# 4m4n5/CLIP-Lite

Hardware: AMD Instinct MI355X
Metric: image-caption pairs/sec (global batch) — ResNet-50+BERT bs1024, 1/2/4/8 MI355X (higher is better)
Workload: dtype bf16; 1 GPU; resnet50 + BERT-base(12L) + JSD-MI heads/priors, per-GPU batch 128, 224x224 images, 30-token captions, dropout 0.1 + prior noise on, clip 10 + SGD(0.9, wd 1e-4) + Lookahead(5, 0.5); global_batch=128, parallelism=dp1

## Files before the change

### clip-lite_amd/bert.py

```python
import torch
import torch.nn as nn

from . import hip


class LinearParams(nn.Module):
    def __init__(self, cin, cout, bias=True, std=None):
        super().__init__()
        self.in_features, self.out_features = cin, cout
        self.weight = nn.Parameter(torch.empty(cout, cin))
        self.bias = nn.Parameter(torch.zeros(cout)) if bias else None
        if std is None:
            nn.init.kaiming_uniform_(self.weight, a=5 ** 0.5)
            if bias:
                bound = 1 / cin ** 0.5
                nn.init.uniform_(self.bias, -bound, bound)
        else:
            self.weight.data.normal_(0.0, std)


class LayerNormParams(nn.Module):
    def __init__(self, c, eps):
        super().__init__()
        self.normalized_shape, self.eps = (c,), eps
# ... 274 lines not shown
        ds2 = _alloc(rt, M, Hd)
        ds2m = _alloc(rt, M, Hd) if d2[0] > 0 else None
        hip.layernorm_bwd(dt, dh, s2, st2, out.LayerNorm.weight, ds2, ds2m, A.g(out.LayerNorm.weight), A.g(out.LayerNorm.bias), M, Hd, drop_out=d2,
                          dcolsum=A.g(out.dense.bias))
        dz2 = ds2m if ds2m is not None else ds2
        _linear_grads(rt, out.dense, dz2, g, M, bias_done=True, defer=defer)
        df = _alloc(rt, M, inner)
        ib = layer.intermediate.dense.bias
        fold = ib is not None and ib.requires_grad
        _dgrad(rt, dz2, M, inner, Hd, hip.epilogue(df, inner, dact_aux=f, dact=hip.DACT_GELU, colsum=A.g(ib) if fold else None, colsum_rows=1),
               out.dense.weight)
        _linear_grads(rt, layer.intermediate.dense, df, h1, M, bias_done=fold, defer=defer)
        dh1 = _alloc(rt, M, Hd)
        _dgrad(rt, df, M, Hd, inner, hip.epilogue(dh1, Hd, residual=ds2), layer.intermediate.dense.weight)
        ds1 = _alloc(rt, M, Hd)
        ds1m = _alloc(rt, M, Hd) if d1[0] > 0 else None
        hip.layernorm_bwd(dt, dh1, s1, st1, ln1.weight, ds1, ds1m, A.g(ln1.weight), A.g(ln1.bias), M, Hd, drop_out=d1,
                          dcolsum=A.g(wo.bias))
        dz1 = ds1m if ds1m is not None else ds1
        _linear_grads(rt, wo, dz1, ctxt, M, bias_done=True, defer=defer)
        dctx = _alloc(rt, M, Hd)
        _dgrad(rt, dz1, M, Hd, Hd, hip.epilogue(dctx, Hd), wo.weight)
        dqkv = _alloc(rt, M, 3 * Hd)
        if mp:
            n_part = B * heads * 32
            hip.attention_bias_bwd(dt, qkv, ctx["mask"], ctx["bias"], net.bucket_table, dctx, dqkv, ctx["dbias_partials"][li * n_part:(li + 1) * n_part],
                                   B, L, heads, da)
        else:
            hip.attention_bwd(dt, qkv, ctx["mask"], dctx, dqkv, B, L, heads, da)
        _linear_grads(rt, None, dqkv, h, M, dw=A.span([wq.weight, wk.weight, wv.weight], grad=True).view(3 * Hd, Hd),
                      db=A.span([wq.bias, wk.bias, wv.bias], grad=True), defer=defer)
        dhp = _alloc(rt, M, Hd)
        _dgrad(rt, dqkv, M, Hd, 3 * Hd, hip.epilogue(dhp, Hd, residual=ds1), wq.weight, wk.weight, wv.weight)
        dh = dhp
        if own_group is None:
            rt.grads_ready(layer)
        elif staged:
            own_group.launch()
            if not pooler_done:
                rt.grads_ready(net.pooler)
                pooler_done = True
            rt.grads_ready(layer)
            defer = own_group = hip.WgradGroup(rt.dt)
    if not last:
        ctx["bwd_dh"] = dh
        return
    emb = net.embeddings
    ds0 = _alloc(rt, M, Hd)
    if mp:
        rel = net.encoder.relative_attention_bias.weight
        if nl and rel.requires_grad:
            hip.attention_bias_grad_reduce(ctx["dbias_partials"], A.g(rel), nl * B, heads)
        if own_group is None or staged:
            rt.grads_ready(net.encoder.relative_attention_bias)
# ... 18 lines not shown
```

### clip-lite_amd/csrc/bert_ops.hip

```cpp
#include "vec.h"
#include "rng.h"
#include "det.h"
#include "clite.h"

using namespace clite;

namespace {

constexpr int LN_MAXCH = 4;

struct Drop { float p; uint64_t seed; uint32_t site; };

DEV void apply_dropout8(const Drop& d, size_t idx, float (&v)[8]) {
  float u[8];
  dropout_uniform8(d.seed, d.site, idx, u);
  float ks = 1.0f / (1.0f - d.p);
#pragma unroll
  for (int e = 0; e < 8; ++e) v[e] = u[e] >= d.p ? v[e] * ks : 0.f;
}

struct LnQ8 { uint8_t* out; const float* scale; float* amax; };
template <typename T, int NCH, bool Q = false>
__global__ __launch_bounds__(256) void layernorm_fwd_kernel(const T* x, const float* gamma, const float* beta, float eps, T* out,
                                                            float* stats, int M, int C, Drop drop, LnQ8 q8) {
// ... 474 lines not shown
      dk += sm.dS[t * AT_PP + r] * sm.f.q[t * AT_PQ + lane];
      dv += sm.f.p[t * AT_PP + r] * sm.f.m[t * AT_PP + r] * sm.dO[t * AT_PQ + lane];
    }
    dq *= 0.125f; dk *= 0.125f;
    T* o = obase + (size_t)r * ld + lane;
    if constexpr (sizeof(T) == 2) { o[0] = f2bf(dq); o[H * AT_D] = f2bf(dk); o[2 * H * AT_D] = f2bf(dv); }
    else { o[0] = dq; o[H * AT_D] = dk; o[2 * H * AT_D] = dv; }
  }
}
constexpr int AM_PI = 192;
constexpr int AM_PT = 80;

struct AmFwdSmem { char v[32 * AM_PI]; float madd[32]; };
struct AmBwdSmem { char q[32 * AM_PI], k[32 * AM_PI], d[32 * AM_PI], t[32 * AM_PT]; float m[32 * 33]; float madd[32]; };

DEV void am_load_image(const bf16* base, size_t ld, int L, char* img, int lane) {
  for (int c = lane; c < 256; c += 64) {
    int r = c >> 3, ch = c & 7;
    u32x4 v = {0u, 0u, 0u, 0u};
    if (r < L) v = *(const u32x4*)(base + (size_t)r * ld + ch * 8);
    *(u32x4*)(img + r * AM_PI + ch * 16) = v;
  }
}
DEV bf16x8 am_frag_rows(const bf16* base, size_t ld, int L, int ks, int lane) {
  Chunk16 c;
  c.u = u32x4{0u, 0u, 0u, 0u};
  int r = lane & 31;
  if (r < L) c.u = *(const u32x4*)(base + (size_t)r * ld + ks * 16 + 8 * (lane >> 5));
  return c.h;
}
template <int PITCH> DEV bf16x8 am_frag_tr(const char* img, int x0, int s, int lane) {
  int x = x0 + 16 * ((lane >> 4) & 1) + 4 * (lane & 3);
  int k = 16 * s + 8 * (lane >> 5) + ((lane >> 2) & 3);
  const char* p = img + k * PITCH + x * 2;
  union { s16x4 v[2]; bf16x8 h; } u;
  u.v[0] = lds_read_tr16(p);
  u.v[1] = lds_read_tr16(p + 4 * PITCH);
  return u.h;
}
template <int PITCH> DEV bf16x8 am_frag_tr_acc(const char* img, int x0, int s, int lane) {
  int x = x0 + 16 * ((lane >> 4) & 1) + 4 * (lane & 3);
  int k = 16 * s + 4 * (lane >> 5) + ((lane >> 2) & 3);
  const char* p = img + k * PITCH + x * 2;
  union { s16x4 v[2]; bf16x8 h; } u;
  u.v[0] = lds_read_tr16(p);
  u.v[1] = lds_read_tr16(p + 8 * PITCH);
  return u.h;
}
DEV bf16x8 am_acc_frag(const f32x16& a, int s) {
  bf16x8 f;
#pragma unroll
  for (int e = 0; e < 8; ++e) f[e] = f2bf(a[8 * s + e]);
  return f;
}
DEV int am_row(int r, int lane) { return (r & 3) + 8 * (r >> 2) + 4 * (lane >> 5); }
DEV void am_store_T(bf16* base, size_t ld, int L, int d0, const f32x16& a, float scale, int lane) {
  int tok = lane & 31;
  if (tok >= L) return;
#pragma unroll
  for (int g = 0; g < 4; ++g) {
    union { bf16 e[4]; u32x2 u; } pk;
#pragma unroll
    for (int e = 0; e < 4; ++e) pk.e[e] = f2bf(a[4 * g + e] * scale);
    *(u32x2*)(base + (size_t)tok * ld + d0 + 8 * g + 4 * (lane >> 5)) = pk.u;
  }
}

template <bool BIAS = false>
__global__ __launch_bounds__(256) void attention_mfma_fwd_kernel(const bf16* qkv, const int64_t* mask, bf16* ctx, int B, int L, int H, Drop drop, AttnBias<BIAS> ab) {
  seed_resolve(drop.seed, drop.site);
  __shared__ __attribute__((aligned(16))) AmFwdSmem sm[4];
  const int lane = threadIdx.x & 63, wave = threadIdx.x >> 6;
  int bh = blockIdx.x * 4 + wave;
  const bool live = bh < B * H;
  if (!live) bh = B * H - 1;
  const int b = bh / H, h = bh % H;
  const size_t ld = (size_t)3 * H * 64;
  const bf16* qb = qkv + (size_t)b * L * ld + h * 64;
  AmFwdSmem& S = sm[wave];
  am_load_image(qb + 2 * H * 64, ld, L, S.v, lane);
  if (lane < 32) S.madd[lane] = (lane < L) ? ((mask && mask[(size_t)b * L + lane] == 0) ? AT_NEG : 0.f) : -INFINITY;
  f32x16 acc;
#pragma unroll
  for (int r = 0; r < 16; ++r) acc[r] = 0.f;
#pragma unroll
  for (int ks = 0; ks < 4; ++ks)
    acc = mfma32_bf16(am_frag_rows(qb + H * 64, ld, L, ks, lane), am_frag_rows(qb, ld, L, ks, lane), acc);
// ... 11 lines not shown
  for (int r = 0; r < 16; ++r) { acc[r] = __expf(acc[r] - mx); den += acc[r]; }
  den += wave_shfl_xor(den, 32);
  const float inv = 1.0f / den;
  const int i = lane & 31;
#pragma unroll
  for (int g = 0; g < 4; ++g) {
    float u[4] = {1.f, 1.f, 1.f, 1.f};
    if (drop.p > 0.f) rng_uniform4(drop.seed, drop.site, ((size_t)bh * AT_L + i) * AT_L + 8 * g + 4 * (lane >> 5), u);
    const float ks = drop.p > 0.f ? 1.0f / (1.0f - drop.p) : 1.f;
#pragma unroll
    for (int e = 0; e < 4; ++e) acc[4 * g + e] *= inv * (u[e] >= drop.p ? ks : 0.f);
  }
#pragma unroll
  for (int db = 0; db < 2; ++db) {
    f32x16 o;
#pragma unroll
    for (int r = 0; r < 16; ++r) o[r] = 0.f;
#pragma unroll
    for (int s = 0; s < 2; ++s) o = mfma32_bf16(am_frag_tr_acc<AM_PI>(S.v, db * 32, s, lane), am_acc_frag(acc, s), o);
    if (live) am_store_T(ctx + (size_t)b * L * ((size_t)H * 64) + h * 64, (size_t)H * 64, L, db * 32, o, 1.f, lane);
  }
}
template <bool BIAS = false>
__global__ __launch_bounds__(128) void attention_mfma_bwd_kernel(const bf16* qkv, const int64_t* mask, const bf16* dctx, bf16* dqkv, int B, int L, int H, Drop drop,
                                                                 AttnBias<BIAS> ab) {
  seed_resolve(drop.seed, drop.site);
  __shared__ __attribute__((aligned(16))) AmBwdSmem sm[2];
  const int lane = threadIdx.x & 63, wave = threadIdx.x >> 6;
  int bh = blockIdx.x * 2 + wave;
  const bool live = bh < B * H;
  if (!live) bh = B * H - 1;
  const int b = bh / H, h = bh % H;
  const size_t ld = (size_t)3 * H * 64, ldc = (size_t)H * 64;
  const bf16* qb = qkv + (size_t)b * L * ld + h * 64;
  const bf16* dob = dctx + (size_t)b * L * ldc + h * 64;
  AmBwdSmem& S = sm[wave];
  am_load_image(qb, ld, L, S.q, lane);
  am_load_image(qb + H * 64, ld, L, S.k, lane);
  am_load_image(dob, ldc, L, S.d, lane);
  if (lane < 32) S.madd[lane] = (lane < L) ? ((mask && mask[(size_t)b * L + lane] == 0) ? AT_NEG : 0.f) : -INFINITY;
  {
    const float ks = drop.p > 0.f ? 1.0f / (1.0f - drop.p) : 1.f;
    for (int q4 = lane; q4 < 256; q4 += 64) {
      int i = q4 >> 3, j0 = (q4 & 7) * 4;
      float u[4] = {1.f, 1.f, 1.f, 1.f};
      if (drop.p > 0.f) rng_uniform4(drop.seed, drop.site, ((size_t)bh * AT_L + i) * AT_L + j0, u);
#pragma unroll
      for (int e = 0; e < 4; ++e) S.m[i * 33 + j0 + e] = u[e] >= drop.p ? ks : 0.f;
    }
  }
  f32x16 p, dp;
#pragma unroll
  for (int r = 0; r < 16; ++r) { p[r] = 0.f; dp[r] = 0.f; }
#pragma unroll
  for (int ks = 0; ks < 4; ++ks) {
    p = mfma32_bf16(am_frag_rows(qb, ld, L, ks, lane), am_frag_rows(qb + H * 64, ld, L, ks, lane), p);
    dp = mfma32_bf16(am_frag_rows(dob, ldc, L, ks, lane), am_frag_rows(qb + 2 * H * 64, ld, L, ks, lane), dp);
  }
  __syncthreads();
  const int j = lane & 31;
  const float madd = S.madd[j];
  f32x16 pd, ds;
#pragma unroll
  for (int r = 0; r < 16; ++r) {
    float s;
    if constexpr (BIAS) s = (p[r] * 0.125f + ab.bias[((size_t)h * AT_L + am_row(r, lane)) * AT_L + j]) + madd;
    else s = p[r] * 0.125f + madd;
    float mx = s;
#pragma unroll
    for (int m = 16; m >= 1; m >>= 1) mx = fmaxf(mx, wave_shfl_xor(mx, m));
    float e = __expf(s - mx);
    float den = e;
#pragma unroll
    for (int m = 16; m >= 1; m >>= 1) den += wave_shfl_xor(den, m);
    int i = am_row(r, lane);
    float pr = (i < L) ? e / den : 0.f;
    float mul = S.m[i * 33 + j];
    float dpd = dp[r] * mul;
    float t = dpd * pr;
#pragma unroll
    for (int m = 16; m >= 1; m >>= 1) t += wave_shfl_xor(t, m);
    p[r] = pr;
    pd[r] = pr * mul;
    ds[r] = pr * (dpd - t);
  }
  if constexpr (BIAS) {
#pragma unroll
    for (int r = 0; r < 16; ++r) S.m[am_row(r, lane) * 33 + j] = ds[r];
  }
#pragma unroll
  for (int g = 0; g < 4; ++g) {
    union { bf16 e[4]; u32x2 u; } pk;
#pragma unroll
    for (int e = 0; e < 4; ++e) pk.e[e] = f2bf(ds[4 * g + e]);
    *(u32x2*)(S.t + j * AM_PT + (8 * g + 4 * (lane >> 5)) * 2) = pk.u;
  }
  __syncthreads();
  if constexpr (BIAS) attn_bucket_sums(S.m, 33, L, ab.btab, live ? ab.partials + (size_t)bh * AT_L : nullptr, lane);
  bf16* ob = dqkv + (size_t)b * L * ld + h * 64;
#pragma unroll
  for (int db = 0; db < 2; ++db) {
    f32x16 dv, dk, dq;
#pragma unroll
    for (int r = 0; r < 16; ++r) { dv[r] = 0.f; dk[r] = 0.f; dq[r] = 0.f; }
#pragma unroll
    for (int s = 0; s < 2; ++s) {
      dv = mfma32_bf16(am_frag_tr_acc<AM_PI>(S.d, db * 32, s, lane), am_acc_frag(pd, s), dv);
      dk = mfma32_bf16(am_frag_tr_acc<AM_PI>(S.q, db * 32, s, lane), am_acc_frag(ds, s), dk);
      dq = mfma32_bf16(am_frag_tr<AM_PI>(S.k, db * 32, s, lane), am_frag_tr<AM_PT>(S.t, 0, s, lane), dq);
    }
    if (live) {
      am_store_T(ob + 2 * H * 64, ld, L, db * 32, dv, 1.f, lane);
      am_store_T(ob + H * 64, ld, L, db * 32, dk, 0.125f, lane);
      am_store_T(ob, ld, L, db * 32, dq, 0.125f, lane);
    }
  }
}
__global__ __launch_bounds__(256) void attention_bias_build_kernel(const float* rel, const int32_t* btab, float* bias, int H, int L) {
  const int idx = blockIdx.x * 256 + threadIdx.x;
  if (idx >= H * AT_L * AT_L) return;
  const int h = idx / (AT_L * AT_L), i = (idx / AT_L) % AT_L, j = idx % AT_L;
  float v = 0.f;
  if (i < L && j < L) {
    int k = btab[j - i + AT_L - 1];
    k = k < 0 ? 0 : (k > AT_L - 1 ? AT_L - 1 : k);
    v = rel[k * H + h];
  }
  bias[idx] = v;
}
__global__ __launch_bounds__(1024) void attention_bias_grad_reduce_kernel(const float* partials, float* drel, int R, int H) {
  __shared__ float red[32][33];
  const int h = blockIdx.x, k = threadIdx.x & 31, part = threadIdx.x >> 5;
  float acc = 0.f;
  for (int r = part; r < R; r += 32) acc += partials[((size_t)r * H + h) * AT_L + k];
  red[part][k] = acc;
  __syncthreads();
  if (threadIdx.x < 32) {
    float t = 0.f;
// ... 447 lines not shown
           hipLaunchKernelGGL(embed_bwd_kernel<float>, dim3(egrid), dim3(128), 0, st, ids, (const float*)d, dword, dpos, M / L, L, C, vocab, padding_idx, EmbMp<false>{}));
  return (int)hipGetLastError();
}

extern "C" int clite_attention_fwd(int dtype, const void* qkv, const int64_t* mask, void* ctx, int B, int L, int H,
                                   float drop_p, uint64_t drop_seed, uint32_t drop_site, void* stream) {
  if (B <= 0 || L <= 0 || L > AL_L || H <= 0 || !qkv || !ctx) return -1;
  Drop d{drop_p, drop_seed, drop_site};
  hipStream_t st = (hipStream_t)stream;
  if (L > AT_L) {
#define AL_FWD(NT) hipLaunchKernelGGL(attention_long_mfma_fwd_kernel<NT>, dim3(B * H), dim3(64 * NT), 0, st, (const bf16*)qkv, mask, (bf16*)ctx, B, L, H, d)
    DISPATCH(dtype,
             if (L <= 64) AL_FWD(2); else if (L <= 96) AL_FWD(3); else AL_FWD(4),
             hipLaunchKernelGGL(attention_long_fwd_kernel<float>, dim3(B * H), dim3(256), 0, st, (const float*)qkv, mask, (float*)ctx, B, L, H, d));
#undef AL_FWD
    return (int)hipGetLastError();
  }
  DISPATCH(dtype,
           hipLaunchKernelGGL(attention_mfma_fwd_kernel<false>, dim3((B * H + 3) / 4), dim3(256), 0, st, (const bf16*)qkv, mask, (bf16*)ctx, B, L, H, d, AttnBias<false>{}),
           hipLaunchKernelGGL(attention_fwd_kernel<float>, dim3(B * H), dim3(64), 0, st, (const float*)qkv, mask, (float*)ctx, B, L, H, d, AttnBias<false>{}));
  return (int)hipGetLastError();
}

extern "C" int clite_attention_bwd(int dtype, const void* qkv, const int64_t* mask, const void* dctx, void* dqkv, int B, int L, int H,
                                   float drop_p, uint64_t drop_seed, uint32_t drop_site, void* stream) {
  if (B <= 0 || L <= 0 || L > AL_L || H <= 0 || !qkv || !dctx || !dqkv) return -1;
  Drop d{drop_p, drop_seed, drop_site};
  hipStream_t st = (hipStream_t)stream;
  if (L > AT_L) {
#define AL_BWD(NT) hipLaunchKernelGGL(attention_long_mfma_bwd_kernel<NT>, dim3(B * H), dim3(64 * NT), 0, st, (const bf16*)qkv, mask, (const bf16*)dctx, (bf16*)dqkv, B, L, H, d)
    DISPATCH(dtype,
             if (L <= 64) AL_BWD(2); else if (L <= 96) AL_BWD(3); else AL_BWD(4),
             hipLaunchKernelGGL(attention_long_bwd_kernel<float>, dim3(B * H), dim3(256), 0, st, (const float*)qkv, mask, (const float*)dctx, (float*)dqkv, B, L, H, d));
#undef AL_BWD
    return (int)hipGetLastError();
  }
  DISPATCH(dtype,
           hipLaunchKernelGGL(attention_mfma_bwd_kernel<false>, dim3((B * H + 1) / 2), dim3(128), 0, st, (const bf16*)qkv, mask, (const bf16*)dctx, (bf16*)dqkv, B, L, H, d, AttnBias<false>{}),
           hipLaunchKernelGGL(attention_bwd_kernel<float>, dim3(B * H), dim3(64), 0, st, (const float*)qkv, mask, (const float*)dctx, (float*)dqkv, B, L, H, d, AttnBias<false>{}));
  return (int)hipGetLastError();
}

extern "C" int clite_attention_bias_fwd(int dtype, const void* qkv, const int64_t* mask, const float* bias, void* ctx, int B, int L, int H,
                                        float drop_p, uint64_t drop_seed, uint32_t drop_site, void* stream) {
  if (B <= 0 || L <= 0 || L > AT_L || H <= 0 || !qkv || !ctx || !bias) return -1;
  Drop d{drop_p, drop_seed, drop_site};
  AttnBias<true> ab{bias, nullptr, nullptr};
  hipStream_t st = (hipStream_t)stream;
  DISPATCH(dtype,
           hipLaunchKernelGGL(attention_mfma_fwd_kernel<true>, dim3((B * H + 3) / 4), dim3(256), 0, st, (const bf16*)qkv, mask, (bf16*)ctx, B, L, H, d, ab),
           hipLaunchKernelGGL((attention_fwd_kernel<float, true>), dim3(B * H), dim3(64), 0, st, (const float*)qkv, mask, (float*)ctx, B, L, H, d, ab));
  return (int)hipGetLastError();
}

extern "C" int clite_attention_bias_bwd(int dtype, const void* qkv, const int64_t* mask, const float* bias, const int32_t* bucket_table, const void* dctx,
                                        void* dqkv, float* dbias_partials, int B, int L, int H, float drop_p, uint64_t drop_seed, uint32_t drop_site,
                                        void* stream) {
  if (B <= 0 || L <= 0 || L > AT_L || H <= 0 || !qkv || !dctx || !dqkv || !bias || !bucket_table || !dbias_partials) return -1;
  Drop d{drop_p, drop_seed, drop_site};
  AttnBias<true> ab{bias, bucket_table, dbias_partials};
  hipStream_t st = (hipStream_t)stream;
  DISPATCH(dtype,
           hipLaunchKernelGGL(attention_mfma_bwd_kernel<true>, dim3((B * H + 1) / 2), dim3(128), 0, st, (const bf16*)qkv, mask, (const bf16*)dctx, (bf16*)dqkv, B, L, H, d, ab),
           hipLaunchKernelGGL((attention_bwd_kernel<float, true>), dim3(B * H), dim3(64), 0, st, (const float*)qkv, mask, (const float*)dctx, (float*)dqkv, B, L, H, d, ab));
  return (int)hipGetLastError();
}

extern "C" int clite_attention_bias_build(const float* rel_weight, const int32_t* bucket_table, float* bias, int H, int L, void* stream) {
  if (H <= 0 || L <= 0 || L > AT_L || !rel_weight || !bucket_table || !bias) return -1;
  hipLaunchKernelGGL(attention_bias_build_kernel, dim3((H * AT_L * AT_L + 255) / 256), dim3(256), 0, (hipStream_t)stream, rel_weight, bucket_table, bias, H, L);
  return (int)hipGetLastError();
}

extern "C" int clite_attention_bias_grad_reduce(const float* partials, float* drel, int rows, int H, void* stream) {
  if (rows <= 0 || H <= 0 || !partials || !drel) return -1;
  hipLaunchKernelGGL(attention_bias_grad_reduce_kernel, dim3(H), dim3(1024), 0, (hipStream_t)stream, partials, drel, rows, H);
  return (int)hipGetLastError();
}

extern "C" int clite_embed_mpnet_fwd(int dtype, const int64_t* ids, const void* word, const void* pos, void* out, int32_t* pids, int M, int L, int C,
                                     int vocab, int max_pos, int padding_idx, void* stream) {
  if (M <= 0 || L <= 0 || L > 32 || M % L || C % 8 || vocab <= 0 || max_pos <= 0 || !ids || !word || !pos || !out) return -1;
  int grid = (M + 3) / 4;
  if (grid > 4096) grid = 4096;
  hipStream_t st = (hipStream_t)stream;
  DISPATCH(dtype,
           hipLaunchKernelGGL(embed_mpnet_fwd_kernel<bf16>, dim3(grid), dim3(256), 0, st, ids, (const bf16*)word, (const bf16*)pos, (bf16*)out, pids, M, L, C, vocab, max_pos, padding_idx),
           hipLaunchKernelGGL(embed_mpnet_fwd_kernel<float>, dim3(grid), dim3(256), 0, st, ids, (const float*)word, (const float*)pos, (float*)out, pids, M, L, C, vocab, max_pos, padding_idx));
// ... 46 lines not shown
```

### clip-lite_amd/hip.py

```python
import ctypes as C
import os

import torch

_HERE = os.path.dirname(os.path.abspath(__file__))
LIB_PATH = os.environ.get("CLITE_HIP_LIB") or os.path.join(_HERE, "lib", "libclite_hip.so")
ABI_VERSION = 12

BF16, F32 = 0, 1
ACT_NONE, ACT_RELU, ACT_GELU, ACT_TANH = 0, 1, 2, 3
DACT_RELU, DACT_GELU, DACT_TANH = 1, 2, 3
SEED_INDIRECT = 0x80000000

TORCH_DTYPE = {BF16: torch.bfloat16, F32: torch.float32}


class Epilogue(C.Structure):
    _fields_ = [
        ("out", C.c_void_p), ("ldc", C.c_int32), ("out_f32", C.c_int32), ("atomic", C.c_int32),
        ("alpha", C.c_float), ("bias", C.c_void_p), ("act", C.c_int32), ("preact", C.c_void_p),
        ("dact_aux", C.c_void_p), ("dact", C.c_int32), ("drop_p", C.c_float), ("drop_seed", C.c_uint64),
        ("drop_site", C.c_uint32), ("residual", C.c_void_p), ("colsum", C.c_void_p),
        ("colsum_replicas", C.c_int32), ("colsum_stride", C.c_int32), ("colsum_rows", C.c_int32),
        ("bn_y", C.c_void_p), ("bn_stats", C.c_void_p), ("bn_replicas", C.c_int32), ("bn_rstride", C.c_int32),
# ... 85 lines not shown
    "clite_stem_pack": [_V, _V, _I, _V],
    "clite_stem_unpack_grad": [_V, _V, _V],
    "clite_bn_apply": [_V, _I, _V, _V, _V, _V],
    "clite_bn_centered_var": [_I, _V, _V, _I, _I, _I, _I, _V],
    "clite_bn_bwd_reduce": [_I, _V, _V, _V, _V, _V, _V, _I, _I, _I, _I, _V],
    "clite_bn_bwd_apply": [_V, _I, _V, _V, _V, _V, _V, _V, _V, _V, _V, _V],
    "clite_maxpool3x3s2_fwd": [_I, _V, _V, _V, _I, _I, _I, _I, _V],
    "clite_maxpool3x3s2_bwd": [_I, _V, _V, _V, _I, _I, _I, _I, _V],
    "clite_stem_bn_pool_fwd": [_V, _I, _V, _V, _V, _I, _I, _I, _V],
    "clite_stem_bn_pool_bwd": [_V, _I, _V, _V, _V, _V, _V, _V, _V, _I, _I, _I, _V],
    "clite_stem_bn_pool_fwd_ex": [_V, _I, _V, _V, _V, _V, _I, _I, _I, _V],
    "clite_stem_bn_pool_bwd_apply": [_V, _I, _V, _V, _V, _V, _V, _V, _V, _I, _I, _I, _V],
    "clite_avgpool_fwd": [_I, _V, _V, _I, _I, _I, _V],
    "clite_avgpool_bwd": [_I, _V, _V, _I, _I, _I, _V],
    "clite_image_to_nhwc4": [_I, _V, _V, _I, _I, _I, _I, _I, _I, _V],
    "clite_colsum": [_I, _V, _V, _I, _I, _V],
    "clite_layernorm_fwd": [_I, _V, _V, _V, _F, _V, _V, _I, _I, _F, _U64, _U32, _V],
    "clite_layernorm_fwd_q8": [_I, _V, _V, _V, _F, _V, _V, _I, _I, _F, _U64, _U32, _V, _V, _V, _V],
    "clite_layernorm_bwd": [_I, _V, _V, _V, _V, _V, _V, _V, _V, _V, _I, _I, _F, _U64, _U32, _F, _U64, _U32, _V],
    "clite_embed_fwd": [_I, _V, _V, _V, _V, _V, _I, _I, _I, _I, _V],
    "clite_embed_bwd": [_I, _V, _V, _V, _V, _I, _I, _I, _I, _I, _V],
    "clite_attention_fwd": [_I, _V, _V, _V, _I, _I, _I, _F, _U64, _U32, _V],
    "clite_attention_bwd": [_I, _V, _V, _V, _V, _I, _I, _I, _F, _U64, _U32, _V],
    "clite_attention_bias_fwd": [_I, _V, _V, _V, _V, _I, _I, _I, _F, _U64, _U32, _V],
    "clite_attention_bias_bwd": [_I, _V, _V, _V, _V, _V, _V, _V, _I, _I, _I, _F, _U64, _U32, _V],
    "clite_attention_bias_build": [_V, _V, _V, _I, _I, _V],
    "clite_attention_bias_grad_reduce": [_V, _V, _I, _I, _V],
    "clite_embed_mpnet_fwd": [_I, _V, _V, _V, _V, _V, _I, _I, _I, _I, _I, _I, _V],
    "clite_embed_mpnet_bwd": [_I, _V, _V, _V, _V, _V, _I, _I, _I, _I, _I, _I, _V],
    "clite_mean_pool_fwd": [_I, _V, _V, _V, _V, _I, _I, _I, _V],
    "clite_mean_pool_bwd": [_I, _V, _V, _V, _V, _I, _I, _I, _V],
    "clite_tanh_bwd": [_I, _V, _V, _V, _U64, _V],
    "clite_critic_jsd_fwd": [_I, _V, _V, _V, _I, _I, _V, _V, _V, _V],
    "clite_l2_normalize": [_I, _V, _V, _I, _I, _V],
    "clite_l2_normalize_bwd": [_I, _V, _V, _V, _V, _I, _I, _V],
    "clite_infonce_fwd": [_V, _I, _I, _V, _V, _V, _V, _V],
    "clite_infonce_bwd": [_I, _V, _I, _I, _V, _V, _V, _V, _F, _V, _I, _V, _V],
    "clite_xent_fwd": [_V, _I, _I, _I, _V, _I, _V, _V, _V],
    "clite_xent_bwd": [_I, _V, _I, _I, _I, _I, _V, _V, _V, _V, _V, _I, _V],
    "clite_svm_margin": [_V, _V, _V, _I, _I, _I, _V, _V, _V, _V, _V],
    "clite_svm_hess_scale": [_V, _V, _U64, _V],
    "clite_svm_newton_begin": [_V, _I, _I, _I, _V, _V, _V, _V, _F, _I, _F, _V],
    "clite_svm_cg_update": [_V, _I, _I, _I, _V, _V, _V, _V, _V],
    "clite_svm_line_search": [_V, _V, _V, _V, _I, _I, _I, _V, _V, _I, _I, _V, _V],
    "clite_average_precision": [_V, _I, _V, _I, _I, _I, _V, _V],
    "clite_retrieval_rank_i2t": [_V, _I, _I, _I, _V, _V, _V, _V],
    "clite_retrieval_rank_t2i": [_V, _I, _I, _I, _V, _V, _V, _V],
    "clite_kmeans_row_norms": [_V, _I, _I, _I, _F, _V, _V],
# ... 570 lines not shown
                                           p(fp8[0]), p(fp8[1]), p(fp8[2]), stream_ptr(x)), "layernorm_fwd_q8")
        return
    check(lib().clite_layernorm_fwd(dt, p(x), p(gamma), p(beta), eps, p(out), p(stats), M, Cc, drop[0], drop[1], drop[2], stream_ptr(x)),
          "layernorm_fwd")


def layernorm_bwd(dt, dy, x, stats, gamma, dx, dx_masked, dgamma, dbeta, M, Cc, drop_in=NO_DROP, drop_out=NO_DROP, dcolsum=None):
    check(lib().clite_layernorm_bwd(dt, p(dy), p(x), p(stats), p(gamma), p(dx), p(dx_masked), p(dgamma), p(dbeta), p(dcolsum), M, Cc,
                                    drop_in[0], drop_in[1], drop_in[2], drop_out[0], drop_out[1], drop_out[2], stream_ptr(x)), "layernorm_bwd")


def embed_fwd(dt, ids, word, pos, typ, out, M, L, Cc, vocab):
    check(lib().clite_embed_fwd(dt, p(ids), p(word), p(pos), p(typ), p(out), M, L, Cc, vocab, stream_ptr(out)), "embed_fwd")


def embed_bwd(dt, ids, d, dword, dpos, M, L, Cc, vocab, padding_idx=-1):
    check(lib().clite_embed_bwd(dt, p(ids), p(d), p(dword), p(dpos), M, L, Cc, vocab, padding_idx, stream_ptr(d)), "embed_bwd")


def attention_fwd(dt, qkv, mask, ctx, B, L, H, drop=NO_DROP):
    check(lib().clite_attention_fwd(dt, p(qkv), p(mask), p(ctx), B, L, H, drop[0], drop[1], drop[2], stream_ptr(qkv)), "attention_fwd")


def attention_bwd(dt, qkv, mask, dctx, dqkv, B, L, H, drop=NO_DROP):
    check(lib().clite_attention_bwd(dt, p(qkv), p(mask), p(dctx), p(dqkv), B, L, H, drop[0], drop[1], drop[2], stream_ptr(qkv)), "attention_bwd")


def relative_position_buckets(num_buckets=32, max_distance=128, span=31):
    half = num_buckets // 2
    exact = half // 2
    assert (num_buckets, max_distance) == (32, 128), "the closed form below is for MPNetConfig's defaults"
    out = []
    for rel in range(-span, span + 1):
        n = -rel
        ret = half if n < 0 else 0
        n = abs(n)
        if n < exact:
            ret += n
        else:
            t = 0
            while 2 ** (t + 1) * exact * exact <= n * n:
                t += 1
            ret += min(exact + t, half - 1)
        out.append(ret)
    return out


def attention_bias_fwd(dt, qkv, mask, bias, ctx, B, L, H, drop=NO_DROP):
    check(lib().clite_attention_bias_fwd(dt, p(qkv), p(mask), p(bias), p(ctx), B, L, H, drop[0], drop[1], drop[2], stream_ptr(qkv)), "attention_bias_fwd")


def attention_bias_bwd(dt, qkv, mask, bias, table, dctx, dqkv, partials, B, L, H, drop=NO_DROP):
    assert partials.dtype == torch.float32 and partials.numel() >= B * H * 32 and table.dtype == torch.int32 and table.numel() == 63
    check(lib().clite_attention_bias_bwd(dt, p(qkv), p(mask), p(bias), p(table), p(dctx), p(dqkv), p(partials), B, L, H, drop[0], drop[1], drop[2],
                                         stream_ptr(qkv)), "attention_bias_bwd")


def attention_bias_build(rel_weight, table, bias, H, L):
    assert rel_weight.dtype == torch.float32 and tuple(rel_weight.shape) == (32, H) and bias.dtype == torch.float32 and bias.numel() == H * 1024
    assert table.dtype == torch.int32 and table.numel() == 63
    check(lib().clite_attention_bias_build(p(rel_weight), p(table), p(bias), H, L, stream_ptr(bias)), "attention_bias_build")


def attention_bias_grad_reduce(partials, drel, rows, H):
    assert partials.numel() >= rows * H * 32 and drel.dtype == torch.float32 and drel.numel() == 32 * H
    check(lib().clite_attention_bias_grad_reduce(p(partials), p(drel), rows, H, stream_ptr(partials)), "attention_bias_grad_reduce")


def embed_mpnet_fwd(dt, ids, word, pos, out, pids, M, L, Cc, vocab, max_pos, padding_idx):
    check(lib().clite_embed_mpnet_fwd(dt, p(ids), p(word), p(pos), p(out), p(pids), M, L, Cc, vocab, max_pos, padding_idx, stream_ptr(out)), "embed_mpnet_fwd")


def embed_mpnet_bwd(dt, ids, pids, d, dword, dpos, M, L, Cc, vocab, max_pos, padding_idx):
    check(lib().clite_embed_mpnet_bwd(dt, p(ids), p(pids), p(d), p(dword), p(dpos), M, L, Cc, vocab, max_pos, padding_idx, stream_ptr(d)), "embed_mpnet_bwd")


def mean_pool_fwd(dt, h, mask, out, inv, B, L, Cc):
    check(lib().clite_mean_pool_fwd(dt, p(h), p(mask), p(out), p(inv), B, L, Cc, stream_ptr(out)), "mean_pool_fwd")
# ... 271 lines not shown
```

### include/clite.h

```cpp
#ifndef CLITE_H
#define CLITE_H
#include <stdint.h>

#ifdef __cplusplus
extern "C" {
#endif

#define CLITE_ABI_VERSION 12
int clite_abi_version(void);

int clite_set_deterministic(int on);
int clite_get_deterministic(void);

int clite_set_f32_split(int on);
int clite_get_f32_split(void);

int clite_set_tile_policy(int policy);

enum { CLITE_BF16 = 0, CLITE_F32 = 1 };

#define CLITE_SEED_INDIRECT 0x80000000u

enum { CLITE_ACT_NONE = 0, CLITE_ACT_RELU = 1, CLITE_ACT_GELU = 2, CLITE_ACT_TANH = 3 };

// ... 182 lines not shown
int clite_stem_bn_pool_bwd_apply(const clite_bn* p, int dtype, const void* dpool, const uint8_t* idx, const void* y, const float* dstats, void* dy,
                                 float* dgamma, float* dbeta, int N, int H, int W, void* stream);
int clite_avgpool_fwd(int dtype, const void* x, void* out, int N, int HW, int C, void* stream);
int clite_avgpool_bwd(int dtype, const void* dout, void* dx, int N, int HW, int C, void* stream);
int clite_image_to_nhwc4(int dtype, const float* img, void* out, int N, int H, int W, int pad, int Hp, int Wp, void* stream);
int clite_colsum(int dtype, const void* x, float* out, int M, int N, void* stream);

int clite_layernorm_fwd(int dtype, const void* x, const float* gamma, const float* beta, float eps, void* out, float* stats,
                        int M, int C, float drop_p, uint64_t drop_seed, uint32_t drop_site, void* stream);
int clite_layernorm_fwd_q8(int dtype, const void* x, const float* gamma, const float* beta, float eps, void* out, float* stats,
                           int M, int C, float drop_p, uint64_t drop_seed, uint32_t drop_site, uint8_t* fp8_out, const float* fp8_scale, float* fp8_amax,
                           void* stream);
int clite_layernorm_bwd(int dtype, const void* dy, const void* x, const float* stats, const float* gamma, void* dx, void* dx_masked,
                        float* dgamma, float* dbeta, float* dcolsum, int M, int C, float in_p, uint64_t in_seed, uint32_t in_site,
                        float out_p, uint64_t out_seed, uint32_t out_site, void* stream);
int clite_embed_fwd(int dtype, const int64_t* ids, const void* word, const void* pos, const void* type, void* out,
                    int M, int L, int C, int vocab, void* stream);
int clite_embed_bwd(int dtype, const int64_t* ids, const void* d, float* dword, float* dpos, int M, int L, int C, int vocab, int padding_idx,
                    void* stream);
int clite_attention_fwd(int dtype, const void* qkv, const int64_t* mask, void* ctx, int B, int L, int H,
                        float drop_p, uint64_t drop_seed, uint32_t drop_site, void* stream);
int clite_attention_bwd(int dtype, const void* qkv, const int64_t* mask, const void* dctx, void* dqkv, int B, int L, int H,
                        float drop_p, uint64_t drop_seed, uint32_t drop_site, void* stream);

int clite_attention_bias_fwd(int dtype, const void* qkv, const int64_t* mask, const float* bias, void* ctx, int B, int L, int H,
                             float drop_p, uint64_t drop_seed, uint32_t drop_site, void* stream);
int clite_attention_bias_bwd(int dtype, const void* qkv, const int64_t* mask, const float* bias, const int32_t* bucket_table, const void* dctx,
                             void* dqkv, float* dbias_partials, int B, int L, int H, float drop_p, uint64_t drop_seed, uint32_t drop_site,
                             void* stream);
int clite_attention_bias_build(const float* rel_weight, const int32_t* bucket_table, float* bias, int H, int L, void* stream);
int clite_attention_bias_grad_reduce(const float* partials, float* drel, int rows, int H, void* stream);
int clite_embed_mpnet_fwd(int dtype, const int64_t* ids, const void* word, const void* pos, void* out, int32_t* pids, int M, int L, int C,
                          int vocab, int max_pos, int padding_idx, void* stream);
int clite_embed_mpnet_bwd(int dtype, const int64_t* ids, const int32_t* pids, const void* d, float* dword, float* dpos, int M, int L, int C,
                          int vocab, int max_pos, int padding_idx, void* stream);
int clite_mean_pool_fwd(int dtype, const void* h, const int64_t* mask, void* out, float* inv, int B, int L, int C, void* stream);
int clite_mean_pool_bwd(int dtype, const void* dy, const int64_t* mask, const float* inv, void* dh, int B, int L, int C, void* stream);

int clite_tanh_bwd(int dtype, const void* dy, const void* y, void* out, uint64_t n, void* stream);

int clite_critic_jsd_fwd(int dtype, const void* f1, const void* f2, const float* temperature, int B, int D, const int32_t* neg, float* work,
                         float* acc, void* stream);
int clite_l2_normalize(int dtype, const void* x, void* out, int B, int D, void* stream);
int clite_l2_normalize_bwd(int dtype, const void* x, const void* y, const void* dy, void* dx, int B, int D, void* stream);
int clite_infonce_fwd(const float* C, int ld, int B, const float* temperature, float* lse_r, float* lse_c, float* acc, void* stream);
int clite_infonce_bwd(int dtype, const float* C, int ld, int B, const float* temperature, const float* lse_r, const float* lse_c,
                      const float* gout, float scale, void* dC, int ldd, float* dtemp, void* stream);
int clite_critic_jsd_bwd(int dtype, const void* f1, const void* f2, const float* temperature, const float* work, const float* gout, float scale,
                         int B, int D, const int32_t* neg, const int32_t* neg_inv, void* df1, void* df2, float* dtemp, void* stream);
int clite_prior_tail_fwd(int dtype, const void* h1, const float* w2, const float* b2, int B, int K, int softplus, float* logit, float* acc,
                         void* stream);
int clite_prior_tail_bwd(int dtype, const void* h1, const float* w2, const float* logit, const float* gout, float scale, int B, int K,
// ... 98 lines not shown
```

Measured before the change: 8782 pairs/s.

## Fuse QKV bias-gradient reduction into attention backward kernel and prefetch operands

The attention backward kernel now stages the finished dQ/dK/dV tiles in LDS, sums them over tokens, and atomically adds the result into the fused QKV bias gradient. This lets the separate bias reduction in the linear-grad path be skipped. The kernel also prefetches Q, K, dO, V fragments, the mask and the bias values into registers before the dropout mask generation, then feeds the MFMAs from LDS images instead of re-reading global memory. This adds float atomics, which are non-deterministic, so the fused path is disabled in deterministic mode. It also raises register pressure.

Result: no change. 8841 pairs/s (median of 6 runs) (+0.7%).

```diff
diff --git a/clip-lite_amd/bert.py b/clip-lite_amd/bert.py
--- a/clip-lite_amd/bert.py
+++ b/clip-lite_amd/bert.py
@@ -320,14 +320,16 @@
         dctx = _alloc(rt, M, Hd)
         _dgrad(rt, dz1, M, Hd, Hd, hip.epilogue(dctx, Hd), wo.weight)
         dqkv = _alloc(rt, M, 3 * Hd)
+        qkv_db = A.span([wq.bias, wk.bias, wv.bias], grad=True)
+        fused_db = qkv_db is not None and hip.attention_dbias_applies(dt, L)
         if mp:
             n_part = B * heads * 32
             hip.attention_bias_bwd(dt, qkv, ctx["mask"], ctx["bias"], net.bucket_table, dctx, dqkv, ctx["dbias_partials"][li * n_part:(li + 1) * n_part],
-                                   B, L, heads, da)
-        else:
-            hip.attention_bwd(dt, qkv, ctx["mask"], dctx, dqkv, B, L, heads, da)
+                                   B, L, heads, da, dqkv_bias=qkv_db if fused_db else None)
+        else:
+            hip.attention_bwd(dt, qkv, ctx["mask"], dctx, dqkv, B, L, heads, da, dqkv_bias=qkv_db if fused_db else None)
         _linear_grads(rt, None, dqkv, h, M, dw=A.span([wq.weight, wk.weight, wv.weight], grad=True).view(3 * Hd, Hd),
-                      db=A.span([wq.bias, wk.bias, wv.bias], grad=True), defer=defer)
+                      db=None if fused_db else qkv_db, defer=defer)
         dhp = _alloc(rt, M, Hd)
         _dgrad(rt, dqkv, M, Hd, 3 * Hd, hip.epilogue(dhp, Hd, residual=ds1), wq.weight, wk.weight, wv.weight)
         dh = dhp
diff --git a/clip-lite_amd/csrc/bert_ops.hip b/clip-lite_amd/csrc/bert_ops.hip
--- a/clip-lite_amd/csrc/bert_ops.hip
+++ b/clip-lite_amd/csrc/bert_ops.hip
@@ -520,6 +520,34 @@
     *(u32x4*)(img + r * AM_PI + ch * 16) = v;
   }
 }
+DEV void am_fetch_image(const bf16* base, size_t ld, int L, u32x4 (&g)[4], int lane) {
+#pragma unroll
+  for (int n = 0; n < 4; ++n) {
+    int c = lane + 64 * n, r = c >> 3, ch = c & 7;
+    g[n] = *(const u32x4*)(base + (size_t)(r < L ? r : 0) * ld + ch * 8);
+  }
+}
+DEV void am_store_image(const u32x4 (&g)[4], int L, char* img, int lane) {
+#pragma unroll
+  for (int n = 0; n < 4; ++n) {
+    int c = lane + 64 * n, r = c >> 3;
+    *(u32x4*)(img + r * AM_PI + (c & 7) * 16) = r < L ? g[n] : u32x4{0u, 0u, 0u, 0u};
+  }
+}
+DEV u32x4 am_fetch_frag_rows(const bf16* base, size_t ld, int L, int ks, int lane) {
+  int r = lane & 31;
+  return *(const u32x4*)(base + (size_t)(r < L ? r : 0) * ld + ks * 16 + 8 * (lane >> 5));
+}
+DEV bf16x8 am_frag_fetched(u32x4 g, int L, int lane) {
+  Chunk16 c;
+  c.u = (lane & 31) < L ? g : u32x4{0u, 0u, 0u, 0u};
+  return c.h;
+}
+DEV bf16x8 am_frag_img(const char* img, int ks, int lane) {
+  Chunk16 c;
+  c.u = *(const u32x4*)(img + (lane & 31) * AM_PI + ks * 32 + 16 * (lane >> 5));
+  return c.h;
+}
 DEV bf16x8 am_frag_rows(const bf16* base, size_t ld, int L, int ks, int lane) {
   Chunk16 c;
   c.u = u32x4{0u, 0u, 0u, 0u};
@@ -561,6 +589,17 @@
 #pragma unroll
     for (int e = 0; e < 4; ++e) pk.e[e] = f2bf(a[4 * g + e] * scale);
     *(u32x2*)(base + (size_t)tok * ld + d0 + 8 * g + 4 * (lane >> 5)) = pk.u;
+  }
+}
+DEV void am_stash_T(char* img, int L, int d0, const f32x16& a, float scale, int lane) {
+  int tok = lane & 31;
+  if (tok >= L) return;
+#pragma unroll
+  for (int g = 0; g < 4; ++g) {
+    union { bf16 e[4]; u32x2 u; } pk;
+#pragma unroll
+    for (int e = 0; e < 4; ++e) pk.e[e] = f2bf(a[4 * g + e] * scale);
+    *(u32x2*)(img + tok * AM_PI + (d0 + 8 * g + 4 * (lane >> 5)) * 2) = pk.u;
   }
 }
 
@@ -618,8 +657,8 @@
   }
 }
 template <bool BIAS = false>
-__global__ __launch_bounds__(128) void attention_mfma_bwd_kernel(const bf16* qkv, const int64_t* mask, const bf16* dctx, bf16* dqkv, int B, int L, int H, Drop drop,
-                                                                 AttnBias<BIAS> ab) {
+__global__ __launch_bounds__(128) void attention_mfma_bwd_kernel(const bf16* qkv, const int64_t* mask, const bf16* dctx, bf16* dqkv, float* dqkv_bias, int B, int L,
+                                                                 int H, Drop drop, AttnBias<BIAS> ab) {
   seed_resolve(drop.seed, drop.site);
   __shared__ __attribute__((aligned(16))) AmBwdSmem sm[2];
   const int lane = threadIdx.x & 63, wave = threadIdx.x >> 6;
@@ -631,36 +670,59 @@
   const bf16* qb = qkv + (size_t)b * L * ld + h * 64;
   const bf16* dob = dctx + (size_t)b * L * ldc + h * 64;
   AmBwdSmem& S = sm[wave];
-  am_load_image(qb, ld, L, S.q, lane);
-  am_load_image(qb + H * 64, ld, L, S.k, lane);
-  am_load_image(dob, ldc, L, S.d, lane);
-  if (lane < 32) S.madd[lane] = (lane < L) ? ((mask && mask[(size_t)b * L + lane] == 0) ? AT_NEG : 0.f) : -INFINITY;
+  u32x4 gq[4], gk[4], gd[4];
+  am_fetch_image(qb, ld, L, gq, lane);
+  am_fetch_image(qb + H * 64, ld, L, gk, lane);
+  am_fetch_image(dob, ldc, L, gd, lane);
+  u32x4 gv[4];
+#pragma unroll
+  for (int ks = 0; ks < 4; ++ks) gv[ks] = am_fetch_frag_rows(qb + 2 * H * 64, ld, L, ks, lane);
+  u32x2 gm = {1u, 0u};
+  if (mask) gm = *(const u32x2*)(mask + (size_t)b * L + (lane < L ? lane : 0));
+  float bs[BIAS ? 16 : 1];
+  if constexpr (BIAS) {
+#pragma unroll
+    for (int r = 0; r < 16; ++r) bs[r] = ab.bias[((size_t)h * AT_L + am_row(r, lane)) * AT_L + (lane & 31)];
+  }
   {
     const float ks = drop.p > 0.f ? 1.0f / (1.0f - drop.p) : 1.f;
-    for (int q4 = lane; q4 < 256; q4 += 64) {
-      int i = q4 >> 3, j0 = (q4 & 7) * 4;
-      float u[4] = {1.f, 1.f, 1.f, 1.f};
-      if (drop.p > 0.f) rng_uniform4(drop.seed, drop.site, ((size_t)bh * AT_L + i) * AT_L + j0, u);
-#pragma unroll
-      for (int e = 0; e < 4; ++e) S.m[i * 33 + j0 + e] = u[e] >= drop.p ? ks : 0.f;
-    }
-  }
+    float u[4][4];
+#pragma unroll
+    for (int n = 0; n < 4; ++n) {
+      int q4 = lane + 64 * n, i = q4 >> 3, j0 = (q4 & 7) * 4;
+#pragma unroll
+      for (int e = 0; e < 4; ++e) u[n][e] = 1.f;
+      if (drop.p > 0.f) rng_uniform4(drop.seed, drop.site, ((size_t)bh * AT_L + i) * AT_L + j0, u[n]);
+    }
+#pragma unroll
+    for (int n = 0; n < 4; ++n) {
+      int q4 = lane + 64 * n, i = q4 >> 3, j0 = (q4 & 7) * 4;
+#pragma unroll
+      for (int e = 0; e < 4; ++e) S.m[i * 33 + j0 + e] = u[n][e] >= drop.p ? ks : 0.f;
+    }
+  }
+  am_store_image(gq, L, S.q, lane);
+  am_store_image(gk, L, S.k, lane);
+  am_store_image(gd, L, S.d, lane);
+  int m0 = (int)gm[0], m1 = (int)gm[1];
+  opaque_i(m0); opaque_i(m1);
+  if (lane < 32) S.madd[lane] = (lane < L) ? ((m0 | m1) == 0 ? AT_NEG : 0.f) : -INFINITY;
+  __syncthreads();
   f32x16 p, dp;
 #pragma unroll
   for (int r = 0; r < 16; ++r) { p[r] = 0.f; dp[r] = 0.f; }
 #pragma unroll
   for (int ks = 0; ks < 4; ++ks) {
-    p = mfma32_bf16(am_frag_rows(qb, ld, L, ks, lane), am_frag_rows(qb + H * 64, ld, L, ks, lane), p);
-    dp = mfma32_bf16(am_frag_rows(dob, ldc, L, ks, lane), am_frag_rows(qb + 2 * H * 64, ld, L, ks, lane), dp);
-  }
-  __syncthreads();
+    p = mfma32_bf16(am_frag_img(S.q, ks, lane), am_frag_img(S.k, ks, lane), p);
+    dp = mfma32_bf16(am_frag_img(S.d, ks, lane), am_frag_fetched(gv[ks], L, lane), dp);
+  }
   const int j = lane & 31;
   const float madd = S.madd[j];
   f32x16 pd, ds;
 #pragma unroll
   for (int r = 0; r < 16; ++r) {
     float s;
-    if constexpr (BIAS) s = (p[r] * 0.125f + ab.bias[((size_t)h * AT_L + am_row(r, lane)) * AT_L + j]) + madd;
+    if constexpr (BIAS) s = (p[r] * 0.125f + bs[r]) + madd;
     else s = p[r] * 0.125f + madd;
     float mx = s;
 #pragma unroll
@@ -694,22 +756,52 @@
   __syncthreads();
   if constexpr (BIAS) attn_bucket_sums(S.m, 33, L, ab.btab, live ? ab.partials + (size_t)bh * AT_L : nullptr, lane);
   bf16* ob = dqkv + (size_t)b * L * ld + h * 64;
+  f32x16 dv[2], dk[2], dq[2];
 #pragma unroll
   for (int db = 0; db < 2; ++db) {
-    f32x16 dv, dk, dq;
-#pragma unroll
-    for (int r = 0; r < 16; ++r) { dv[r] = 0.f; dk[r] = 0.f; dq[r] = 0.f; }
+#pragma unroll
+    for (int r = 0; r < 16; ++r) { dv[db][r] = 0.f; dk[db][r] = 0.f; dq[db][r] = 0.f; }
 #pragma unroll
     for (int s = 0; s < 2; ++s) {
-      dv = mfma32_bf16(am_frag_tr_acc<AM_PI>(S.d, db * 32, s, lane), am_acc_frag(pd, s), dv);
-      dk = mfma32_bf16(am_frag_tr_acc<AM_PI>(S.q, db * 32, s, lane), am_acc_frag(ds, s), dk);
-      dq = mfma32_bf16(am_frag_tr<AM_PI>(S.k, db * 32, s, lane), am_frag_tr<AM_PT>(S.t, 0, s, lane), dq);
+      dv[db] = mfma32_bf16(am_frag_tr_acc<AM_PI>(S.d, db * 32, s, lane), am_acc_frag(pd, s), dv[db]);
+      dk[db] = mfma32_bf16(am_frag_tr_acc<AM_PI>(S.q, db * 32, s, lane), am_acc_frag(ds, s), dk[db]);
+      dq[db] = mfma32_bf16(am_frag_tr<AM_PI>(S.k, db * 32, s, lane), am_frag_tr<AM_PT>(S.t, 0, s, lane), dq[db]);
     }
     if (live) {
-      am_store_T(ob + 2 * H * 64, ld, L, db * 32, dv, 1.f, lane);
-      am_store_T(ob + H * 64, ld, L, db * 32, dk, 0.125f, lane);
-      am_store_T(ob, ld, L, db * 32, dq, 0.125f, lane);
-    }
+      am_store_T(ob + 2 * H * 64, ld, L, db * 32, dv[db], 1.f, lane);
+      am_store_T(ob + H * 64, ld, L, db * 32, dk[db], 0.125f, lane);
+      am_store_T(ob, ld, L, db * 32, dq[db], 0.125f, lane);
+    }
+  }
+  if (!dqkv_bias) return;
+  lds_barrier();
+#pragma unroll
+  for (int db = 0; db < 2; ++db) {
+    am_stash_T(S.d, L, db * 32, dv[db], 1.f, lane);
+    am_stash_T(S.k, L, db * 32, dk[db], 0.125f, lane);
+    am_stash_T(S.q, L, db * 32, dq[db], 0.125f, lane);
+  }
+  lds_barrier();
+  float cs[3] = {0.f, 0.f, 0.f};
+  for (int t = 0; t < L; ++t) {
+    cs[0] += bf2f(*(const bf16*)(S.q + t * AM_PI + lane * 2));
+    cs[1] += bf2f(*(const bf16*)(S.k + t * AM_PI + lane * 2));
+    cs[2] += bf2f(*(const bf16*)(S.d + t * AM_PI + lane * 2));
+  }
+  if (H == 1) {
+    float* fold = sm[1].m;
+    if (wave == 1) {
+#pragma unroll
+      for (int w = 0; w < 3; ++w) fold[w * 64 + lane] = live ? cs[w] : 0.f;
+    }
+    lds_barrier();
+    if (wave == 1) return;
+#pragma unroll
+    for (int w = 0; w < 3; ++w) cs[w] += fold[w * 64 + lane];
+  }
+  if (live) {
+#pragma unroll
+    for (int w = 0; w < 3; ++w) atomic_add_f32(dqkv_bias + ((size_t)w * H + h) * 64 + lane, cs[w]);
   }
 }
 __global__ __launch_bounds__(256) void attention_bias_build_kernel(const float* rel, const int32_t* btab, float* bias, int H, int L) {
@@ -1203,9 +1295,13 @@
   return (int)hipGetLastError();
 }
 
-extern "C" int clite_attention_bwd(int dtype, const void* qkv, const int64_t* mask, const void* dctx, void* dqkv, int B, int L, int H,
-                                   float drop_p, uint64_t drop_seed, uint32_t drop_site, void* stream) {
-  if (B <= 0 || L <= 0 || L > AL_L || H <= 0 || !qkv || !dctx || !dqkv) return -1;
+static bool attn_dbias_ok(int dtype, int L, const float* dqkv_bias) {
+  return !dqkv_bias || (dtype == CLITE_BF16 && L <= AT_L && !clite::deterministic());
+}
+
+static int attention_bwd_launch(int dtype, const void* qkv, const int64_t* mask, const void* dctx, void* dqkv, float* dqkv_bias, int B, int L, int H,
+                                float drop_p, uint64_t drop_seed, uint32_t drop_site, void* stream) {
+  if (B <= 0 || L <= 0 || L > AL_L || H <= 0 || !qkv || !dctx || !dqkv || !attn_dbias_ok(dtype, L, dqkv_bias)) return -1;
   Drop d{drop_p, drop_seed, drop_site};
   hipStream_t st = (hipStream_t)stream;
   if (L > AT_L) {
@@ -1217,9 +1313,19 @@
     return (int)hipGetLastError();
   }
   DISPATCH(dtype,
-           hipLaunchKernelGGL(attention_mfma_bwd_kernel<false>, dim3((B * H + 1) / 2), dim3(128), 0, st, (const bf16*)qkv, mask, (const bf16*)dctx, (bf16*)dqkv, B, L, H, d, AttnBias<false>{}),
+           hipLaunchKernelGGL(attention_mfma_bwd_kernel<false>, dim3((B * H + 1) / 2), dim3(128), 0, st, (const bf16*)qkv, mask, (const bf16*)dctx, (bf16*)dqkv, dqkv_bias, B, L, H, d, AttnBias<false>{}),
            hipLaunchKernelGGL(attention_bwd_kernel<float>, dim3(B * H), dim3(64), 0, st, (const float*)qkv, mask, (const float*)dctx, (float*)dqkv, B, L, H, d, AttnBias<false>{}));
   return (int)hipGetLastError();
+}
+
+extern "C" int clite_attention_bwd(int dtype, const void* qkv, const int64_t* mask, const void* dctx, void* dqkv, int B, int L, int H,
+                                   float drop_p, uint64_t drop_seed, uint32_t drop_site, void* stream) {
+  return attention_bwd_launch(dtype, qkv, mask, dctx, dqkv, nullptr, B, L, H, drop_p, drop_seed, drop_site, stream);
+}
+
+extern "C" int clite_attention_bwd_dbias(int dtype, const void* qkv, const int64_t* mask, const void* dctx, void* dqkv, float* dqkv_bias, int B, int L, int H,
+                                         float drop_p, uint64_t drop_seed, uint32_t drop_site, void* stream) {
+  return attention_bwd_launch(dtype, qkv, mask, dctx, dqkv, dqkv_bias, B, L, H, drop_p, drop_seed, drop_site, stream);
 }
 
 extern "C" int clite_attention_bias_fwd(int dtype, const void* qkv, const int64_t* mask, const float* bias, void* ctx, int B, int L, int H,
@@ -1234,17 +1340,30 @@
   return (int)hipGetLastError();
 }
 
-extern "C" int clite_attention_bias_bwd(int dtype, const void* qkv, const int64_t* mask, const float* bias, const int32_t* bucket_table, const void* dctx,
-                                        void* dqkv, float* dbias_partials, int B, int L, int H, float drop_p, uint64_t drop_seed, uint32_t drop_site,
-                                        void* stream) {
+static int attention_bias_bwd_launch(int dtype, const void* qkv, const int64_t* mask, const float* bias, const int32_t* bucket_table, const void* dctx,
+                                     void* dqkv, float* dbias_partials, float* dqkv_bias, int B, int L, int H, float drop_p, uint64_t drop_seed,
+                                     uint32_t drop_site, void* stream) {
   if (B <= 0 || L <= 0 || L > AT_L || H <= 0 || !qkv || !dctx || !dqkv || !bias || !bucket_table || !dbias_partials) return -1;
+  if (!attn_dbias_ok(dtype, L, dqkv_bias)) return -1;
   Drop d{drop_p, drop_seed, drop_site};
   AttnBias<true> ab{bias, bucket_table, dbias_partials};
   hipStream_t st = (hipStream_t)stream;
   DISPATCH(dtype,
-           hipLaunchKernelGGL(attention_mfma_bwd_kernel<true>, dim3((B * H + 1) / 2), dim3(128), 0, st, (const bf16*)qkv, mask, (const bf16*)dctx, (bf16*)dqkv, B, L, H, d, ab),
+           hipLaunchKernelGGL(attention_mfma_bwd_kernel<true>, dim3((B * H + 1) / 2), dim3(128), 0, st, (const bf16*)qkv, mask, (const bf16*)dctx, (bf16*)dqkv, dqkv_bias, B, L, H, d, ab),
            hipLaunchKernelGGL((attention_bwd_kernel<float, true>), dim3(B * H), dim3(64), 0, st, (const float*)qkv, mask, (const float*)dctx, (float*)dqkv, B, L, H, d, ab));
   return (int)hipGetLastError();
+}
+
+extern "C" int clite_attention_bias_bwd(int dtype, const void* qkv, const int64_t* mask, const float* bias, const int32_t* bucket_table, const void* dctx,
+                                        void* dqkv, float* dbias_partials, int B, int L, int H, float drop_p, uint64_t drop_seed, uint32_t drop_site,
+                                        void* stream) {
+  return attention_bias_bwd_launch(dtype, qkv, mask, bias, bucket_table, dctx, dqkv, dbias_partials, nullptr, B, L, H, drop_p, drop_seed, drop_site, stream);
+}
+
+extern "C" int clite_attention_bias_bwd_dbias(int dtype, const void* qkv, const int64_t* mask, const float* bias, const int32_t* bucket_table, const void* dctx,
+                                              void* dqkv, float* dbias_partials, float* dqkv_bias, int B, int L, int H, float drop_p, uint64_t drop_seed,
+                                              uint32_t drop_site, void* stream) {
+  return attention_bias_bwd_launch(dtype, qkv, mask, bias, bucket_table, dctx, dqkv, dbias_partials, dqkv_bias, B, L, H, drop_p, drop_seed, drop_site, stream);
 }
 
 extern "C" int clite_attention_bias_build(const float* rel_weight, const int32_t* bucket_table, float* bias, int H, int L, void* stream) {
diff --git a/clip-lite_amd/hip.py b/clip-lite_amd/hip.py
--- a/clip-lite_amd/hip.py
+++ b/clip-lite_amd/hip.py
@@ -131,8 +131,10 @@
     "clite_embed_bwd": [_I, _V, _V, _V, _V, _I, _I, _I, _I, _I, _V],
     "clite_attention_fwd": [_I, _V, _V, _V, _I, _I, _I, _F, _U64, _U32, _V],
     "clite_attention_bwd": [_I, _V, _V, _V, _V, _I, _I, _I, _F, _U64, _U32, _V],
+    "clite_attention_bwd_dbias": [_I, _V, _V, _V, _V, _V, _I, _I, _I, _F, _U64, _U32, _V],
     "clite_attention_bias_fwd": [_I, _V, _V, _V, _V, _I, _I, _I, _F, _U64, _U32, _V],
     "clite_attention_bias_bwd": [_I, _V, _V, _V, _V, _V, _V, _V, _I, _I, _I, _F, _U64, _U32, _V],
+    "clite_attention_bias_bwd_dbias": [_I, _V, _V, _V, _V, _V, _V, _V, _V, _I, _I, _I, _F, _U64, _U32, _V],
     "clite_attention_bias_build": [_V, _V, _V, _I, _I, _V],
     "clite_attention_bias_grad_reduce": [_V, _V, _I, _I, _V],
     "clite_embed_mpnet_fwd": [_I, _V, _V, _V, _V, _V, _I, _I, _I, _I, _I, _I, _V],
@@ -749,8 +751,17 @@
     check(lib().clite_attention_fwd(dt, p(qkv), p(mask), p(ctx), B, L, H, drop[0], drop[1], drop[2], stream_ptr(qkv)), "attention_fwd")
 
 
-def attention_bwd(dt, qkv, mask, dctx, dqkv, B, L, H, drop=NO_DROP):
-    check(lib().clite_attention_bwd(dt, p(qkv), p(mask), p(dctx), p(dqkv), B, L, H, drop[0], drop[1], drop[2], stream_ptr(qkv)), "attention_bwd")
+def attention_dbias_applies(dt, L):
+    return dt == BF16 and L <= 32 and not is_deterministic()
+
+
+def attention_bwd(dt, qkv, mask, dctx, dqkv, B, L, H, drop=NO_DROP, dqkv_bias=None):
+    if dqkv_bias is None:
+        check(lib().clite_attention_bwd(dt, p(qkv), p(mask), p(dctx), p(dqkv), B, L, H, drop[0], drop[1], drop[2], stream_ptr(qkv)), "attention_bwd")
+        return
+    assert dqkv_bias.dtype == torch.float32 and dqkv_bias.numel() == 3 * H * 64 and dqkv_bias.is_contiguous()
+    check(lib().clite_attention_bwd_dbias(dt, p(qkv), p(mask), p(dctx), p(dqkv), p(dqkv_bias), B, L, H, drop[0], drop[1], drop[2], stream_ptr(qkv)),
+          "attention_bwd_dbias")
 
 
 def relative_position_buckets(num_buckets=32, max_distance=128, span=31):
@@ -777,10 +788,15 @@
     check(lib().clite_attention_bias_fwd(dt, p(qkv), p(mask), p(bias), p(ctx), B, L, H, drop[0], drop[1], drop[2], stream_ptr(qkv)), "attention_bias_fwd")
 
 
-def attention_bias_bwd(dt, qkv, mask, bias, table, dctx, dqkv, partials, B, L, H, drop=NO_DROP):
+def attention_bias_bwd(dt, qkv, mask, bias, table, dctx, dqkv, partials, B, L, H, drop=NO_DROP, dqkv_bias=None):
     assert partials.dtype == torch.float32 and partials.numel() >= B * H * 32 and table.dtype == torch.int32 and table.numel() == 63
-    check(lib().clite_attention_bias_bwd(dt, p(qkv), p(mask), p(bias), p(table), p(dctx), p(dqkv), p(partials), B, L, H, drop[0], drop[1], drop[2],
-                                         stream_ptr(qkv)), "attention_bias_bwd")
+    if dqkv_bias is None:
+        check(lib().clite_attention_bias_bwd(dt, p(qkv), p(mask), p(bias), p(table), p(dctx), p(dqkv), p(partials), B, L, H, drop[0], drop[1], drop[2],
+                                             stream_ptr(qkv)), "attention_bias_bwd")
+        return
+    assert dqkv_bias.dtype == torch.float32 and dqkv_bias.numel() == 3 * H * 64 and dqkv_bias.is_contiguous()
+    check(lib().clite_attention_bias_bwd_dbias(dt, p(qkv), p(mask), p(bias), p(table), p(dctx), p(dqkv), p(partials), p(dqkv_bias), B, L, H,
+                                               drop[0], drop[1], drop[2], stream_ptr(qkv)), "attention_bias_bwd_dbias")
 
 
 def attention_bias_build(rel_weight, table, bias, H, L):
diff --git a/include/clite.h b/include/clite.h
--- a/include/clite.h
+++ b/include/clite.h
@@ -228,12 +228,17 @@
                         float drop_p, uint64_t drop_seed, uint32_t drop_site, void* stream);
 int clite_attention_bwd(int dtype, const void* qkv, const int64_t* mask, const void* dctx, void* dqkv, int B, int L, int H,
                         float drop_p, uint64_t drop_seed, uint32_t drop_site, void* stream);
+int clite_attention_bwd_dbias(int dtype, const void* qkv, const int64_t* mask, const void* dctx, void* dqkv, float* dqkv_bias, int B, int L, int H,
+                              float drop_p, uint64_t drop_seed, uint32_t drop_site, void* stream);
 
 int clite_attention_bias_fwd(int dtype, const void* qkv, const int64_t* mask, const float* bias, void* ctx, int B, int L, int H,
                              float drop_p, uint64_t drop_seed, uint32_t drop_site, void* stream);
 int clite_attention_bias_bwd(int dtype, const void* qkv, const int64_t* mask, const float* bias, const int32_t* bucket_table, const void* dctx,
                              void* dqkv, float* dbias_partials, int B, int L, int H, float drop_p, uint64_t drop_seed, uint32_t drop_site,
                              void* stream);
+int clite_attention_bias_bwd_dbias(int dtype, const void* qkv, const int64_t* mask, const float* bias, const int32_t* bucket_table, const void* dctx,
+                                   void* dqkv, float* dbias_partials, float* dqkv_bias, int B, int L, int H, float drop_p, uint64_t drop_seed,
+                                   uint32_t drop_site, void* stream);
 int clite_attention_bias_build(const float* rel_weight, const int32_t* bucket_table, float* bias, int H, int L, void* stream);
 int clite_attention_bias_grad_reduce(const float* partials, float* drel, int rows, int H, void* stream);
 int clite_embed_mpnet_fwd(int dtype, const int64_t* ids, const void* word, const void* pos, void* out, int32_t* pids, int M, int L, int C,
```
